# gregbugaj/marie-icr

Hardware: AMD Instinct MI355X
Metric: pages/sec (2550x3300, ~40 lines/page) (higher is better)
Workload: dtype f16; 1 GPU; BASELINE configs[2]: full detect->crop->recognize, 64 synthetic 2550x3300x3 u8 pages per GPU per step resident in HBM; DiT-base Mask R-CNN detector (resize to 1035x800, 1 pass, 8 pages per forward) + TrOCR-base recognizer on the generator's 40 ground-truth line boxes per page (fixed work), beam 3, 15+1 decoder steps; seeded random weights; f16 operands with fp32 accumulation is the 16-bit mode of ; crops_per_page=40

## Files before the change

marie_icr_amd/csrc/cross_attn.hip:

```cpp
#include <math.h>

#include "common.h"

namespace {

typedef _Float16 half8v __attribute__((ext_vector_type(8)));
typedef _Float16 half4v __attribute__((ext_vector_type(4)));
typedef __fp16 fp16x4 __attribute__((__vector_size__(4 * sizeof(__fp16))));
typedef float float4v __attribute__((ext_vector_type(4)));

#ifndef CA_E_AUX
#define CA_E_AUX 2
#endif
__device__ __forceinline__ void glds16(const void* gsrc, void* lds_wave_base) {
  __builtin_amdgcn_global_load_lds((const __attribute__((address_space(1))) void*)gsrc,
                                   (__attribute__((address_space(3))) void*)lds_wave_base, 16, 0, CA_E_AUX);
}
__device__ __forceinline__ half4v lds_tr16(const char* p) {
  fp16x4 v = __builtin_amdgcn_ds_read_tr16_b64_v4f16((__attribute__((address_space(3))) fp16x4*)p);
  return __builtin_bit_cast(half4v, v);
}
__device__ __forceinline__ int swz(int row) { return ((row & 7) << 1) | ((row >> 3) & 1); }

template <int N>
__device__ __forceinline__ void wait_vm() {
  asm volatile("s_waitcnt vmcnt(%0)" ::"n"(N) : "memory");
}
template <int PER, int MAXT>
__device__ __forceinline__ void wait_vm_dyn(int tiles) {
  if constexpr (MAXT <= 0 || PER <= 0) {
    wait_vm<0>();
  } else {
    if (tiles >= MAXT) wait_vm<PER * MAXT>();
    else wait_vm_dyn<PER, MAXT - 1>(tiles);
  }
}

struct CrossArgs {
  const _Float16* E;
  const _Float16* qt;
  _Float16* ct;
  size_t crop_stride, tile_stride;
  int n_keys, heads;
};

#ifndef CA_TK
#define CA_TK 32
#endif
constexpr int TK = CA_TK;
static_assert(TK == 16 || TK == 32, "cross_attn key tile");
static_assert(TK <= CROSS_ATTN_SLACK_ROWS, "the last key tile of the last crop stays inside the slack rows of E");
constexpr int RT = TK / 16;
constexpr int cross_slots(int ed, int w) {
  const int n = (160 * 1024 - 4 * w * 1024) / (TK * ed * 2);
  return n > 6 ? 6 : n;
}

template <int ED, int W, int NPW, int NI, bool FEED>
__device__ __forceinline__ void cross_tile(const char* __restrict__ sb, char* __restrict__ feed_dst, float4v* __restrict__ xb,
                                           const char* __restrict__ feed_src, const int (&dma_off)[NPW],
                                           const int (&a_off)[4], const int (&t_off)[8], const half8v (&qf)[ED / 64],
                                           float4v (&acc)[ED / 32], float& mref, float& lsum, int t, int n_keys, int wave, int lane) {
  constexpr int NW = 2 * W, ROWB = ED * 2, KS = ED / 64, MT = ED / 32;
  const int g = lane >> 4;
#ifdef CA_DMA_ONLY
    if (FEED) {
#pragma unroll
      for (int j = 0; j < NPW; ++j) {
        const int i = wave + j * NW;
        if (NI % NW == 0 || i < NI) glds16(feed_src + dma_off[j], feed_dst + i * 1024);
      }
    }
    if (CA_DMA_ONLY) __builtin_amdgcn_s_barrier();
    return;
#endif
    float4v s[2] = {(float4v){0.f, 0.f, 0.f, 0.f}, (float4v){0.f, 0.f, 0.f, 0.f}};
    constexpr int EVERY = (KS / NPW) > 0 ? (KS / NPW) : 1;
    constexpr int AHEAD = KS < 4 ? KS : 4;
    half8v a0[KS], a1[RT == 2 ? KS : 1];
#pragma unroll
    for (int ks = 0; ks < AHEAD; ++ks) {
      a0[ks] = *(const half8v*)(sb + a_off[ks & 3] + 256 * (ks >> 2));
      if (RT == 2) a1[ks] = *(const half8v*)(sb + a_off[ks & 3] + 256 * (ks >> 2) + 16 * ROWB);
    }
    __builtin_amdgcn_sched_barrier(0);
#pragma unroll
    for (int ks = 0; ks < KS; ++ks) {
      if (ks + AHEAD < KS) {
        a0[ks + AHEAD] = *(const half8v*)(sb + a_off[(ks + AHEAD) & 3] + 256 * ((ks + AHEAD) >> 2));
        if (RT == 2) a1[ks + AHEAD] = *(const half8v*)(sb + a_off[(ks + AHEAD) & 3] + 256 * ((ks + AHEAD) >> 2) + 16 * ROWB);
      }
      if (FEED && ks % EVERY == 0 && ks / EVERY < NPW) {
        const int j = ks / EVERY, i = wave + j * NW;
        if (NI % NW == 0 || i < NI) glds16(feed_src + dma_off[j], feed_dst + i * 1024);
      }
      __builtin_amdgcn_sched_barrier(0);
      s[0] = __builtin_amdgcn_mfma_f32_16x16x32_f16(a0[ks], qf[ks], s[0], 0, 0, 0);
      if (RT == 2) s[1] = __builtin_amdgcn_mfma_f32_16x16x32_f16(a1[RT == 2 ? ks : 0], qf[ks], s[1], 0, 0, 0);
      __builtin_amdgcn_sched_barrier(0);
    }
    if (FEED) {
#pragma unroll
      for (int j = (KS + EVERY - 1) / EVERY; j < NPW; ++j) {
        const int i = wave + j * NW;
        if (NI % NW == 0 || i < NI) glds16(feed_src + dma_off[j], feed_dst + i * 1024);
      }
    }
    xb[(wave * 2 + 0) * 64 + lane] = s[0];
    if (RT == 2) xb[(wave * 2 + 1) * 64 + lane] = s[1];
    __builtin_amdgcn_s_waitcnt(0xc07f);
    __builtin_amdgcn_s_barrier();
    s[0] += xb[((wave ^ 1) * 2 + 0) * 64 + lane];
    if (RT == 2) s[1] += xb[((wave ^ 1) * 2 + 1) * 64 + lane];
    const int key0 = t * TK;
    if (key0 + TK > n_keys) {
#pragma unroll
      for (int mt = 0; mt < RT; ++mt)
#pragma unroll
        for (int e = 0; e < 4; ++e)
          if (key0 + 16 * mt + 4 * g + e >= n_keys) s[mt][e] = -INFINITY;
    }
    float mx = fmaxf(fmaxf(s[0][0], s[0][1]), fmaxf(s[0][2], s[0][3]));
    if (RT == 2) mx = fmaxf(mx, fmaxf(fmaxf(s[1][0], s[1][1]), fmaxf(s[1][2], s[1][3])));
    mx = fmaxf(mx, __shfl_xor(mx, 16));
    mx = fmaxf(mx, __shfl_xor(mx, 32));
    if (t == 0) {
      mref = mx;
    } else if (__builtin_amdgcn_ballot_w64(mx > mref + 8.f) != 0) {
      const float nr = fmaxf(mref, mx), f = __builtin_amdgcn_exp2f(mref - nr);
      mref = nr;
      lsum *= f;
#pragma unroll
      for (int i = 0; i < MT; ++i) acc[i] *= f;
    }
    half8v pf = (half8v){0, 0, 0, 0, 0, 0, 0, 0};
#pragma unroll
    for (int mt = 0; mt < RT; ++mt)
#pragma unroll
      for (int e = 0; e < 4; ++e) {
        const float pe = __builtin_amdgcn_exp2f(s[mt][e] - mref);
        lsum += pe;
        pf[mt * 4 + e] = (_Float16)pe;
      }
    constexpr int TAHEAD = MT < 6 ? MT : 6;
    half4v tlo[MT], thi[RT == 2 ? MT : 1];
    const half4v pf4 = __builtin_shufflevector(pf, pf, 0, 1, 2, 3);
#pragma unroll
    for (int mt = 0; mt < TAHEAD; ++mt) {
      tlo[mt] = lds_tr16(sb + t_off[mt & 7] + 256 * (mt >> 3));
      if (RT == 2) thi[mt] = lds_tr16(sb + t_off[mt & 7] + 256 * (mt >> 3) + 16 * ROWB);
    }
    __builtin_amdgcn_sched_barrier(0);
#pragma unroll
    for (int mt = 0; mt < MT; ++mt) {
      if (mt + TAHEAD < MT) {
        tlo[mt + TAHEAD] = lds_tr16(sb + t_off[(mt + TAHEAD) & 7] + 256 * ((mt + TAHEAD) >> 3));
        if (RT == 2) thi[mt + TAHEAD] = lds_tr16(sb + t_off[(mt + TAHEAD) & 7] + 256 * ((mt + TAHEAD) >> 3) + 16 * ROWB);
      }
      __builtin_amdgcn_sched_barrier(0);
      if constexpr (RT == 2) {
        const half8v a = __builtin_shufflevector(tlo[mt], thi[mt], 0, 1, 2, 3, 4, 5, 6, 7);
        acc[mt] = __builtin_amdgcn_mfma_f32_16x16x32_f16(a, pf, acc[mt], 0, 0, 0);
      } else {
        acc[mt] = __builtin_amdgcn_mfma_f32_16x16x16f16(tlo[mt], pf4, acc[mt], 0, 0, 0);
      }
      __builtin_amdgcn_sched_barrier(0);
    }
}

template <int ED, int W>
__global__ __launch_bounds__(128 * W) void cross_attn_kernel(CrossArgs p) {
  extern __shared__ __attribute__((aligned(16))) char smem[];
  constexpr int NW = 2 * W;
  constexpr int ROWB = ED * 2;
  constexpr int HB = ED;
  constexpr int TILE_B = TK * ROWB;
  constexpr int NS = cross_slots(ED, W);
  constexpr int NI = TILE_B / 1024;
  constexpr int NPW = (NI + NW - 1) / NW;
  constexpr int KS = ED / 64, MT = ED / 32;
  const int tid = threadIdx.x, lane = tid & 63;
  const int wave = __builtin_amdgcn_readfirstlane(tid >> 6);
  const int beam = wave >> 1, hh = wave & 1;
  const int n = lane & 15, g = lane >> 4;
  const int crop = blockIdx.x;
  const char* Ec = (const char*)p.E + (size_t)crop * p.crop_stride;
  const int ntiles = (p.n_keys + TK - 1) / TK;
  float4v* xbuf = (float4v*)(smem + NS * TILE_B);

  int dma_off[NPW];
#pragma unroll
  for (int j = 0; j < NPW; ++j) {
    const int i = wave + j * NW;
    const int byte = i * 1024 + lane * 16;
    const int r = byte / ROWB, cp = (byte - r * ROWB) >> 4;
    const int c = (cp & ~15) | ((cp & 15) ^ swz(r));
    dma_off[j] = r * ROWB + c * 16;
  }
  auto issue = [&](int t, int slot) {
    const char* src = Ec + (size_t)t * p.tile_stride;
    char* dst = smem + slot * TILE_B;
#pragma unroll
    for (int j = 0; j < NPW; ++j) {
      const int i = wave + j * NW;
      if (NI % NW == 0 || i < NI) glds16(src + dma_off[j], dst + i * 1024);
    }
  };
  const bool short_wave = (NI % NW != 0) && (wave + (NPW - 1) * NW >= NI);

  half8v qf[KS];
  {
    const _Float16* qr = p.qt + ((size_t)(crop * W + beam) * 16 + n) * ED + hh * (ED / 2) + g * 8;
#pragma unroll
    for (int ks = 0; ks < KS; ++ks) {
      if (n < p.heads) qf[ks] = *(const half8v*)(qr + ks * 32);
      else qf[ks] = (half8v){0, 0, 0, 0, 0, 0, 0, 0};
    }
  }
  int a_off[4];
#pragma unroll
  for (int j = 0; j < 4; ++j) a_off[j] = n * ROWB + hh * HB + 16 * ((4 * j + g) ^ swz(n));
  int t_off[8];
  {
    const int q = n >> 2, pp = n & 3, row = 4 * g + q, x = swz(row);
#pragma unroll
    for (int j = 0; j < 8; ++j) t_off[j] = row * ROWB + hh * HB + 32 * (j ^ (x >> 1)) + 16 * ((pp >> 1) ^ (x & 1)) + 8 * (pp & 1);
  }

  float4v acc[MT];
#pragma unroll
  for (int i = 0; i < MT; ++i) acc[i] = (float4v){0.f, 0.f, 0.f, 0.f};
  float mref = 0.f, lsum = 0.f;

  constexpr int DEPTH = NS - 1;
  static_assert(NS >= 2 && DEPTH * NPW <= 60, "ring depth / vmcnt range");
#pragma unroll
  for (int i = 0; i < DEPTH; ++i)
    if (i < ntiles) issue(i, i);
  int slot = 0;
  const int nfeed = ntiles > DEPTH ? ntiles - DEPTH : 0;
  for (int t = 0; t < nfeed; ++t) {
    if (short_wave) wait_vm<(NPW - 1) * (DEPTH - 1)>();
    else wait_vm<NPW * (DEPTH - 1)>();
    __builtin_amdgcn_s_barrier();
    const char* feed_src = Ec + (size_t)(t + DEPTH) * p.tile_stride;
    char* feed_dst = smem + (slot == 0 ? NS - 1 : slot - 1) * TILE_B;
    cross_tile<ED, W, NPW, NI, true>(smem + slot * TILE_B, feed_dst, xbuf, feed_src, dma_off, a_off, t_off, qf, acc, mref, lsum, t,
                                     p.n_keys, wave, lane);
    slot = (slot == NS - 1) ? 0 : slot + 1;
  }
  for (int t = nfeed; t < ntiles; ++t) {
    const int after = min(DEPTH - 1, ntiles - 1 - t);
    if (short_wave) wait_vm_dyn<NPW - 1, DEPTH - 1>(after);
    else wait_vm_dyn<NPW, DEPTH - 1>(after);
    __builtin_amdgcn_s_barrier();
    cross_tile<ED, W, NPW, NI, false>(smem + slot * TILE_B, smem, xbuf, Ec, dma_off, a_off, t_off, qf, acc, mref, lsum, t, p.n_keys,
                                      wave, lane);
    slot = (slot == NS - 1) ? 0 : slot + 1;
  }
  lsum += __shfl_xor(lsum, 16);
  lsum += __shfl_xor(lsum, 32);
  const float inv = 1.f / lsum;
  if (n < p.heads) {
    _Float16* o = p.ct + ((size_t)(crop * W + beam) * 16 + n) * ED + hh * (ED / 2) + 4 * g;
#pragma unroll
    for (int mt = 0; mt < MT; ++mt) {
      half4v h;
#pragma unroll
      for (int e = 0; e < 4; ++e) h[e] = (_Float16)(acc[mt][e] * inv);
      *(half4v*)(o + 16 * mt) = h;
    }
  }
}

template <int ED>
__global__ __launch_bounds__(256) void absorb_q_kernel(const _Float16* __restrict__ q, int ldq, const _Float16* __restrict__ wkt,
                                                      _Float16* __restrict__ qt, int rows) {
  __shared__ __attribute__((aligned(16))) _Float16 stage[4][64][72];
  const int lane = threadIdx.x & 63, wave = threadIdx.x >> 6, n = lane & 15, g = lane >> 4;
  const int h = blockIdx.y, r0 = blockIdx.x * 64;
  half8v b[4][2];
#pragma unroll
  for (int nt = 0; nt < 4; ++nt)
#pragma unroll
    for (int ks = 0; ks < 2; ++ks) {
      const int r = r0 + nt * 16 + n;
      if (r < rows) b[nt][ks] = *(const half8v*)(q + (size_t)r * ldq + h * 64 + ks * 32 + g * 8);
      else b[nt][ks] = (half8v){0, 0, 0, 0, 0, 0, 0, 0};
    }
  constexpr int MTW = ED / 64;
  const _Float16* wrow = wkt + ((size_t)h * ED + wave * (ED / 4) + n) * 64 + g * 8;
#pragma unroll 1
  for (int mg = 0; mg < MTW / 4; ++mg) {
#pragma unroll
    for (int mi = 0; mi < 4; ++mi) {
      const int mt = mg * 4 + mi;
      const half8v a0 = *(const half8v*)(wrow + (size_t)mt * 16 * 64);
      const half8v a1 = *(const half8v*)(wrow + (size_t)mt * 16 * 64 + 32);
#pragma unroll
      for (int nt = 0; nt < 4; ++nt) {
        float4v c = {0.f, 0.f, 0.f, 0.f};
        c = __builtin_amdgcn_mfma_f32_16x16x32_f16(a0, b[nt][0], c, 0, 0, 0);
        c = __builtin_amdgcn_mfma_f32_16x16x32_f16(a1, b[nt][1], c, 0, 0, 0);
        half4v o;
#pragma unroll
        for (int e = 0; e < 4; ++e) o[e] = (_Float16)c[e];
        *(half4v*)&stage[wave][nt * 16 + n][mi * 16 + 4 * g] = o;
      }
    }
#pragma unroll
    for (int i = 0; i < 8; ++i) {
      const int row = i * 8 + (lane >> 3), ch = lane & 7, r = r0 + row;
      const uint4 v = *(const uint4*)&stage[wave][row][ch * 8];
      if (r < rows) *(uint4*)(qt + ((size_t)r * 16 + h) * ED + wave * (ED / 4) + mg * 64 + ch * 8) = v;
    }
  }
}

template <int ED>
__global__ __launch_bounds__(256) void absorb_v_kernel(const _Float16* __restrict__ ct, const _Float16* __restrict__ wv,
                                                      const float* __restrict__ bv, _Float16* __restrict__ ao, int ldo, int rows) {
  __shared__ __attribute__((aligned(16))) float4v part[4][16][64];
  const int lane = threadIdx.x & 63, wave = threadIdx.x >> 6, n = lane & 15, g = lane >> 4;
  const int h = blockIdx.y, r0 = blockIdx.x * 64;
  constexpr int KSW = ED / 32 / 4;
  const _Float16* brow[4];
#pragma unroll
  for (int nt = 0; nt < 4; ++nt) brow[nt] = ct + ((size_t)min(r0 + nt * 16 + n, rows - 1) * 16 + h) * ED + wave * (ED / 4) + g * 8;
  const _Float16* arow = wv + ((size_t)h * 64 + n) * ED + wave * (ED / 4) + g * 8;
  float4v c[4][4];
#pragma unroll
  for (int mt = 0; mt < 4; ++mt)
#pragma unroll
    for (int nt = 0; nt < 4; ++nt) c[mt][nt] = (float4v){0.f, 0.f, 0.f, 0.f};
#pragma unroll 2
  for (int ks = 0; ks < KSW; ++ks) {
    half8v a[4], b[4];
#pragma unroll
    for (int nt = 0; nt < 4; ++nt) b[nt] = *(const half8v*)(brow[nt] + ks * 32);
#pragma unroll
    for (int mt = 0; mt < 4; ++mt) a[mt] = *(const half8v*)(arow + (size_t)mt * 16 * ED + ks * 32);
#pragma unroll
    for (int mt = 0; mt < 4; ++mt)
#pragma unroll
      for (int nt = 0; nt < 4; ++nt) c[mt][nt] = __builtin_amdgcn_mfma_f32_16x16x32_f16(a[mt], b[nt], c[mt][nt], 0, 0, 0);
  }
#pragma unroll
  for (int mt = 0; mt < 4; ++mt)
#pragma unroll
    for (int nt = 0; nt < 4; ++nt) part[wave][mt * 4 + nt][lane] = c[mt][nt];
  __syncthreads();
  const int r = r0 + wave * 16 + n;
#pragma unroll
  for (int mt = 0; mt < 4; ++mt) {
    float4v v = part[0][mt * 4 + wave][lane];
#pragma unroll
    for (int w = 1; w < 4; ++w) v += part[w][mt * 4 + wave][lane];
    const float4v bb = *(const float4v*)(bv + h * 64 + mt * 16 + 4 * g);
    half4v o;
#pragma unroll
    for (int e = 0; e < 4; ++e) o[e] = (_Float16)(v[e] + bb[e]);
    if (r < rows) *(half4v*)(ao + (size_t)r * ldo + h * 64 + mt * 16 + 4 * g) = o;
  }
}

template <int ED>
int launch_ed(mhip_ctx* ctx, const CrossAbsorbDesc& d) {
  const int rows = d.crops * d.beam;
  PROF_LAUNCH(ctx, MHIP_K_DEC_OPS, hipLaunchKernelGGL((absorb_q_kernel<ED>), dim3((rows + 63) / 64, d.heads), dim3(256), 0, ctx->stream,
                                                     (const _Float16*)d.q, d.ldq, (const _Float16*)d.wkt, (_Float16*)d.qt, rows));
  CrossArgs a;
  a.E = (const _Float16*)d.E; a.qt = (const _Float16*)d.qt; a.ct = (_Float16*)d.ct;
  constexpr int TILE_B = TK * ED * 2;
  a.n_keys = d.n_keys; a.heads = d.heads;
  a.crop_stride = (size_t)d.kv_rows * ED * 2; a.tile_stride = TILE_B;
  const size_t lds = (size_t)cross_slots(ED, d.beam) * TILE_B + (size_t)d.beam * 4096;
#define CROSS_LAUNCH(WV)                                                                                                       \
  do {                                                                                                                         \
    static std::once_flag attr;                                                                                                \
    std::call_once(attr, [&] {                                                                                                 \
      (void)hipFuncSetAttribute((const void*)cross_attn_kernel<ED, WV>, hipFuncAttributeMaxDynamicSharedMemorySize, (int)lds); \
    });                                                                                                                        \
    PROF_LAUNCH(ctx, MHIP_K_CROSS_ATTN,                                                                                        \
                hipLaunchKernelGGL((cross_attn_kernel<ED, WV>), dim3(d.crops), dim3(128 * WV), lds, ctx->stream, a));          \
  } while (0)
  switch (d.beam) {
    case 1: CROSS_LAUNCH(1); break;
    case 2: CROSS_LAUNCH(2); break;
    case 3: CROSS_LAUNCH(3); break;
    default: CROSS_LAUNCH(4); break;
  }
#undef CROSS_LAUNCH
  PROF_LAUNCH(ctx, MHIP_K_DEC_OPS, hipLaunchKernelGGL((absorb_v_kernel<ED>), dim3((rows + 63) / 64, d.heads), dim3(256), 0, ctx->stream,
                                                     (const _Float16*)d.ct, (const _Float16*)d.wv, d.bv, (_Float16*)d.ao, d.ldo, rows));
  hipError_t e = hipGetLastError();
  if (e != hipSuccess) return mhip_fail(ctx, MHIP_EHIP, "cross_attn launch: %s", hipGetErrorString(e));
  return 0;
}

}

bool mhip_cross_absorb_supported(int enc_dim, int beam, int heads) {
  return (enc_dim == 256 || enc_dim == 512 || enc_dim == 768 || enc_dim == 1024) && beam >= 1 && beam <= 4 && heads >= 1 && heads <= 16;
}

int mhip_launch_cross_absorbed(mhip_ctx* ctx, const CrossAbsorbDesc& d) {
  if (!d.q || !d.E || !d.wkt || !d.wv || !d.bv || !d.qt || !d.ct || !d.ao || d.crops < 1)
    return mhip_fail(ctx, MHIP_EINVAL, "cross_attn: null operand");
  if (!mhip_cross_absorb_supported(d.enc_dim, d.beam, d.heads) || d.n_keys < 1 || d.kv_rows < d.n_keys || d.ldq % 8 || d.ldo % 4)
    return mhip_fail(ctx, MHIP_EINVAL, "cross_attn: unsupported shape (enc_dim %d, beam %d, heads %d)", d.enc_dim, d.beam, d.heads);
  switch (d.enc_dim) {
    case 256: return launch_ed<256>(ctx, d);
    case 512: return launch_ed<512>(ctx, d);
    case 768: return launch_ed<768>(ctx, d);
    default: return launch_ed<1024>(ctx, d);
  }
}
```

Baseline: 95.95 pages/s.

## Stage absorb_v ct tiles through swizzled LDS with double-buffered prefetch

The absorb_v kernel now loads the ct (B operand) rows as coalesced full 128-byte lines into registers and writes them to a per-wave XOR-swizzled LDS stage. The MFMA B fragments are then read back from LDS instead of being gathered as scattered 16-byte global loads. The A and C fetches are double-buffered one or two k-steps ahead, with sched_barriers to overlap loads with MFMA. The cross-wave reduction skips storing each wave's own tile, which shrinks LDS traffic. The cost is higher register pressure and more LDS use, which may reduce occupancy.

```diff
diff --git a/marie_icr_amd/csrc/cross_attn.hip b/marie_icr_amd/csrc/cross_attn.hip
--- a/marie_icr_amd/csrc/cross_attn.hip
+++ b/marie_icr_amd/csrc/cross_attn.hip
@@ -8,6 +8,7 @@
 typedef _Float16 half4v __attribute__((ext_vector_type(4)));
 typedef __fp16 fp16x4 __attribute__((__vector_size__(4 * sizeof(__fp16))));
 typedef float float4v __attribute__((ext_vector_type(4)));
+typedef unsigned uint4v __attribute__((ext_vector_type(4)));
 
 #ifndef CA_E_AUX
 #define CA_E_AUX 2
@@ -317,45 +318,93 @@
   }
 }
 
+constexpr int AV_WAVE_LDS = 12 * 64 * 16;
+
 template <int ED>
 __global__ __launch_bounds__(256) void absorb_v_kernel(const _Float16* __restrict__ ct, const _Float16* __restrict__ wv,
                                                       const float* __restrict__ bv, _Float16* __restrict__ ao, int ldo, int rows) {
-  __shared__ __attribute__((aligned(16))) float4v part[4][16][64];
-  const int lane = threadIdx.x & 63, wave = threadIdx.x >> 6, n = lane & 15, g = lane >> 4;
+  __shared__ __attribute__((aligned(16))) char smem[4 * AV_WAVE_LDS];
+  const int lane = threadIdx.x & 63, n = lane & 15, g = lane >> 4;
+  const int wave = __builtin_amdgcn_readfirstlane(threadIdx.x >> 6);
   const int h = blockIdx.y, r0 = blockIdx.x * 64;
   constexpr int KSW = ED / 32 / 4;
-  const _Float16* brow[4];
-#pragma unroll
-  for (int nt = 0; nt < 4; ++nt) brow[nt] = ct + ((size_t)min(r0 + nt * 16 + n, rows - 1) * 16 + h) * ED + wave * (ED / 4) + g * 8;
+  constexpr int NP = KSW / 2;
+  static_assert(KSW % 2 == 0, "absorb_v: a wave's share of a row is whole 128-byte lines");
+  char* stage = smem + wave * AV_WAVE_LDS;
+  const _Float16* crow[8];
+  int w_off[8];
+#pragma unroll
+  for (int j = 0; j < 8; ++j) {
+    const int row = 8 * j + (lane >> 3);
+    crow[j] = ct + ((size_t)min(r0 + row, rows - 1) * 16 + h) * ED + wave * (ED / 4) + (lane & 7) * 8;
+    w_off[j] = row * 128 + 16 * ((lane & 7) ^ ((row >> 1) & 7));
+  }
+  int b_off[2];
+#pragma unroll
+  for (int ksl = 0; ksl < 2; ++ksl) b_off[ksl] = n * 128 + 16 * ((4 * ksl + g) ^ (n >> 1));
   const _Float16* arow = wv + ((size_t)h * 64 + n) * ED + wave * (ED / 4) + g * 8;
+  uint4v cr[2][8];
+  half8v a[2][2][4];
+  auto fetch_c = [&](int kp) {
+#pragma unroll
+    for (int j = 0; j < 8; ++j) cr[kp & 1][j] = *(const uint4v*)(crow[j] + kp * 64);
+  };
+  auto fetch_a = [&](int kp) {
+#pragma unroll
+    for (int ksl = 0; ksl < 2; ++ksl)
+#pragma unroll
+      for (int mt = 0; mt < 4; ++mt) a[kp & 1][ksl][mt] = *(const half8v*)(arow + (size_t)mt * 16 * ED + (kp * 2 + ksl) * 32);
+  };
   float4v c[4][4];
 #pragma unroll
   for (int mt = 0; mt < 4; ++mt)
 #pragma unroll
     for (int nt = 0; nt < 4; ++nt) c[mt][nt] = (float4v){0.f, 0.f, 0.f, 0.f};
-#pragma unroll 2
-  for (int ks = 0; ks < KSW; ++ks) {
-    half8v a[4], b[4];
-#pragma unroll
-    for (int nt = 0; nt < 4; ++nt) b[nt] = *(const half8v*)(brow[nt] + ks * 32);
-#pragma unroll
-    for (int mt = 0; mt < 4; ++mt) a[mt] = *(const half8v*)(arow + (size_t)mt * 16 * ED + ks * 32);
-#pragma unroll
-    for (int mt = 0; mt < 4; ++mt)
-#pragma unroll
-      for (int nt = 0; nt < 4; ++nt) c[mt][nt] = __builtin_amdgcn_mfma_f32_16x16x32_f16(a[mt], b[nt], c[mt][nt], 0, 0, 0);
-  }
+
+  fetch_c(0);
+  fetch_a(0);
+  if (NP > 1) fetch_c(1);
+  __builtin_amdgcn_sched_barrier(0);
+#pragma unroll
+  for (int kp = 0; kp < NP; ++kp) {
+#pragma unroll
+    for (int j = 0; j < 8; ++j) *(uint4v*)(stage + w_off[j]) = cr[kp & 1][j];
+    __builtin_amdgcn_sched_barrier(0);
+    if (kp + 1 < NP) fetch_a(kp + 1);
+    __builtin_amdgcn_sched_barrier(0);
+    if (kp + 2 < NP) fetch_c(kp + 2);
+    __builtin_amdgcn_sched_barrier(0);
+#pragma unroll
+    for (int ksl = 0; ksl < 2; ++ksl) {
+      half8v b[4];
+#pragma unroll
+      for (int nt = 0; nt < 4; ++nt) b[nt] = *(const half8v*)(stage + b_off[ksl] + nt * 2048);
+#pragma unroll
+      for (int mt = 0; mt < 4; ++mt)
+#pragma unroll
+        for (int nt = 0; nt < 4; ++nt) c[mt][nt] = __builtin_amdgcn_mfma_f32_16x16x32_f16(a[kp & 1][ksl][mt], b[nt], c[mt][nt], 0, 0, 0);
+    }
+    __builtin_amdgcn_sched_barrier(0);
+  }
+  float4v* part = (float4v*)smem;
 #pragma unroll
   for (int mt = 0; mt < 4; ++mt)
 #pragma unroll
-    for (int nt = 0; nt < 4; ++nt) part[wave][mt * 4 + nt][lane] = c[mt][nt];
+    for (int nt = 0; nt < 4; ++nt)
+      if (nt != wave) part[(wave * 12 + mt * 3 + (nt > wave ? nt - 1 : nt)) * 64 + lane] = c[mt][nt];
   __syncthreads();
   const int r = r0 + wave * 16 + n;
 #pragma unroll
   for (int mt = 0; mt < 4; ++mt) {
-    float4v v = part[0][mt * 4 + wave][lane];
-#pragma unroll
-    for (int w = 1; w < 4; ++w) v += part[w][mt * 4 + wave][lane];
+    const float4v own = wave == 0 ? c[mt][0] : wave == 1 ? c[mt][1] : wave == 2 ? c[mt][2] : c[mt][3];
+    float4v v = own;
+#pragma unroll
+    for (int w = 0; w < 4; ++w) {
+      float4v pw = own;
+      if (w != wave) pw = part[(w * 12 + mt * 3 + (wave > w ? wave - 1 : wave)) * 64 + lane];
+      if (w == 0) v = pw;
+      else v += pw;
+    }
     const float4v bb = *(const float4v*)(bv + h * 64 + mt * 16 + 4 * g);
     half4v o;
 #pragma unroll
```

After: 96.08 pages/s (median of 2 runs). About the same (+0.1%).
